# wenxichen/tensorflow_yolo2

Measured on AMD Instinct MI355X. Metric: images/sec fwd+bwd Darknet-19 416x416, higher is better.
Workload: dtype f16; 1 GPU; YOLO detector train step: darknet19_core + darknet19_detection(30) + get_loss + backward + Adam; image_size=416, batch_per_gpu=64, global_batch=64, S=13, B=2, parallelism=dp1, grad_allreduce=none

## Files before the change

tensorflow_yolo2_amd/csrc/common.h:

```cpp
#pragma once
#include <hip/hip_runtime.h>
#include <stdint.h>

namespace y2 {

typedef _Float16 half_t;
typedef __bf16 bf16_t;

typedef float f32x4 __attribute__((ext_vector_type(4)));
typedef float f32x16 __attribute__((ext_vector_type(16)));
typedef _Float16 f16x8 __attribute__((ext_vector_type(8)));
typedef _Float16 f16x4 __attribute__((ext_vector_type(4)));
typedef __bf16 bf16x8 __attribute__((ext_vector_type(8)));
typedef __bf16 bf16x4 __attribute__((ext_vector_type(4)));
typedef uint32_t u32x4 __attribute__((ext_vector_type(4)));
typedef uint32_t u32x2 __attribute__((ext_vector_type(2)));

#define Y2_DEV __device__ __forceinline__

constexpr int kWave = 64;

template <typename T> struct Elem;

template <> struct Elem<float> {
// ... 147 lines not shown
Y2_DEV float leaky01(float z) { return fmaxf(0.1f * z, z); }
Y2_DEV float leaky_s(float z, float s) { return fmaxf(s * z, z); }
Y2_DEV float leaky_slope_s(float z, float s) { return (s * z >= z) ? s : 1.0f; }
Y2_DEV float leaky01_slope(float z) { return (0.1f * z >= z) ? 0.1f : 1.0f; }

typedef short s16x4 __attribute__((__vector_size__(4 * sizeof(short))));
typedef short s16x8 __attribute__((ext_vector_type(8)));

template <typename T>
Y2_DEV typename Elem<T>::frag tr_frag(const char* p0, const char* p1) {
    s16x4 lo = __builtin_amdgcn_ds_read_tr16_b64_v4i16((__attribute__((address_space(3))) s16x4*)p0);
    s16x4 hi = __builtin_amdgcn_ds_read_tr16_b64_v4i16((__attribute__((address_space(3))) s16x4*)p1);
    s16x8 both = {lo[0], lo[1], lo[2], lo[3], hi[0], hi[1], hi[2], hi[3]};
    return __builtin_bit_cast(typename Elem<T>::frag, both);
}

__host__ __device__ inline size_t bpix(int n, int h, int w, int H, int W) {
    return ((size_t)n * (H + 1) + (size_t)(h + 1)) * (size_t)(W + 1) + (size_t)(w + 1);
}
__host__ __device__ inline size_t bbody_pixels(int N, int H, int W) {
    return (size_t)N * (H + 1) * (W + 1) + (size_t)(W + 1) + 1;
}

Y2_DEV int pool_order_pixel(int q, int H, int W) {
    const int Wo = W >> 1, Ho = H >> 1;
    const int win = q >> 2, d = q & 3;
    const int t = win / Wo, wo = win - t * Wo;
    const int n = t / Ho, ho = t - n * Ho;
    return (n * H + 2 * ho + (d >> 1)) * W + 2 * wo + (d & 1);
}

}
```

tensorflow_yolo2_amd/csrc/conv1_wgrad.hip:

```cpp
#include "common.h"
#include "kernels.h"

namespace y2 {

template <typename T>
__global__ __launch_bounds__(256) void conv1_wgrad_kernel(Conv1WgradArgs a) {
    constexpr int SZ = sizeof(T);
    constexpr int DYP = 32 * SZ;
    constexpr int XP = 4 * SZ;
    extern __shared__ __attribute__((aligned(16))) char smem[];
    const int tid = threadIdx.x, lane = tid & 63;
    const int w = __builtin_amdgcn_readfirstlane(tid >> 6);
    const int Wp = (a.W + 15) & ~15;
    const int dy_bytes = Wp * DYP;
    const int x_bytes = ((Wp + 4) * XP + 15) & ~15;
    char* dy_l = smem;
    char* x_l = smem + dy_bytes;
    const int dy_chunks = dy_bytes / 16, x_chunks = x_bytes / 16;
    const int rows = a.N * a.H;
    const int r32 = lane & 31, hh = lane >> 5;
    const int qq = (lane & 15) >> 2, pp = lane & 3, g1 = (lane >> 4) & 1;

    f32x16 acc1, acc2;
#pragma unroll
// ... 699 lines not shown
    for (int i = tid; i < 48 * 32; i += 1024) {
        const int r = i >> 5, co = i & 31;
        const int kh = r >> 4, e = r & 15, kw = e >> 2, c = e & 3;
        Wp[r][co] = (kw < 3 && c < 3) ? a.W[((kh * 3 + kw) * 3 + c) * 32 + co] : 0.f;
    }
    __syncthreads();
    if (tid >= 27 * 32) return;
    const int co = tid & 31, tc = tid >> 5;
    const int c = tc % 3, kw = (tc / 3) % 3, kh = tc / 9;
    const int r = kh * 16 + kw * 4 + c;
    constexpr int kOnes = 1 * 16 + 1 * 4 + 3;
    const float x1 = G[kOnes][r];
    float gw = 0.f;
    for (int k = 0; k < 48; ++k) gw = fmaf(G[r][k], Wp[k][co], gw);
    const float xy = gw + a.bias[co] * x1;
    const float xdz = total(r * 32 + co);
    const float ka = a.coef[co], kb = a.coef[32 + co];
    a.dW[tc * 32 + co] = (a.scale[co] * xdz - ka * x1 - kb * xy) * a.inv_grad_scale;
}

constexpr int kGram = 48 * 48;
constexpr int kGramMaxBlocks = 768;
template <typename T>
__global__ __launch_bounds__(256, 2) void conv1_gram_kernel(const void* x4, int N, int H, int W, int RT, float* part) {
    static_assert(sizeof(T) == 2, "half-precision modes only (the f32 parity mode keeps the statistics-only conv pass)");
    constexpr int SZ = 2, XP = 4 * SZ;
    constexpr int NTH = 256, NW = 4;
    typedef typename Elem<T>::frag frag_t;
    extern __shared__ __attribute__((aligned(16))) char smem[];
    const int tid = threadIdx.x, lane = tid & 63;
    const int w = __builtin_amdgcn_readfirstlane(tid >> 6);
    const int Wp = (W + 31) & ~31;
    const int x_bytes = ((Wp + 4) * XP + 15) & ~15;
    const int x_chunks = x_bytes / 16;
    const int nrow = RT + 2;
    char* x_l = smem;
    const int Ht = H / RT;
    const int ntile = N * Ht;
    const int g4 = lane >> 4, qq = (lane & 15) >> 2, pp = lane & 3;
    f32x4 gb[6];
#pragma unroll
    for (int k = 0; k < 6; ++k) gb[k] = f32x4{0.f, 0.f, 0.f, 0.f};
    auto stage = [&](int t, int buf) {
        const int n = t / Ht, h0 = (t - n * Ht) * RT;
        const char* xrow = (const char*)x4 + (bpix(n, h0, 0, H, W) - (size_t)(W + 2)) * XP;
        const size_t xpitch = (size_t)(W + 1) * XP;
        char* dst = x_l + buf * nrow * x_bytes;
        for (int kh = 0; kh < nrow; ++kh)
            for (int i0 = w * 64; i0 < x_chunks; i0 += NTH) {
                const int i = i0 + lane;
                if (i < x_chunks) glds16(xrow + kh * xpitch + (size_t)i * 16, dst + kh * x_bytes + i0 * 16);
            }
    };
    const int ngrp = (W + 31) / 32, nitem = ngrp * (RT / 2);
    int buf = 0;
    if ((int)blockIdx.x < ntile) stage(blockIdx.x, 0);
    for (int t = blockIdx.x; t < ntile; t += gridDim.x, buf ^= 1) {
        __syncthreads();
        if (t + (int)gridDim.x < ntile) stage(t + gridDim.x, buf ^ 1);
        const char* xb = x_l + buf * nrow * x_bytes;
        for (int it = w; it < nitem; it += NW) {
            const int s = it % ngrp, r0 = 2 * (it / ngrp);
            const int w0 = s * 32;
            const int pix = w0 + 8 * g4 + qq;
            frag_t X[4], B[4];
#pragma unroll
            for (int q = 0; q < 4; ++q) {
                const char* pa = xb + (r0 + q) * x_bytes + (pix + pp) * XP;
                X[q] = tr_frag<T>(pa, pa + 4 * XP);
                B[q] = X[q];
            }
            if (w0 + 32 > W) {
#pragma unroll
                for (int q = 0; q < 4; ++q)
#pragma unroll
                    for (int j = 0; j < 8; ++j)
                        if (w0 + 8 * g4 + j >= W) B[q][j] = (T)0.f;
            }
#pragma unroll
            for (int r = 0; r < 2; ++r) {
                mma16(gb[0], X[r], B[r]);
                mma16(gb[1], X[r], B[r + 1]);
                mma16(gb[2], X[r], B[r + 2]);
                mma16(gb[3], X[r + 1], B[r + 1]);
                mma16(gb[4], X[r + 1], B[r + 2]);
                mma16(gb[5], X[r + 2], B[r + 2]);
            }
        }
    }
    __syncthreads();
    float* red = (float*)smem;
    {
        float* g = red + w * kGram;
        const int bi[6] = {0, 0, 0, 1, 1, 2}, bj[6] = {0, 1, 2, 1, 2, 2};
#pragma unroll
        for (int k = 0; k < 6; ++k)
#pragma unroll
            for (int q = 0; q < 4; ++q) g[(bi[k] * 16 + 4 * g4 + q) * 48 + bj[k] * 16 + (lane & 15)] = gb[k][q];
    }
    __syncthreads();
    for (int i = tid; i < kGram; i += NTH) {
        const int r = i / 48, c = i % 48;
        const int j = (r / 16 > c / 16) ? c * 48 + r : i;
        part[(size_t)blockIdx.x * kGram + i] = (red[j] + red[kGram + j]) + (red[2 * kGram + j] + red[3 * kGram + j]);
    }
}

__global__ __launch_bounds__(256) void conv1_gram_reduce_kernel(const float* part, int nblocks, float* mid) {
    const int i = blockIdx.x * 256 + threadIdx.x;
    if (i >= kGram) return;
    const int per = (nblocks + kLinMid - 1) / kLinMid;
    const int b0 = blockIdx.y * per;
    int b1 = b0 + per;
    if (b1 > nblocks) b1 = nblocks;
    float v4[4] = {0.f, 0.f, 0.f, 0.f};
    int b = b0;
    for (; b + 3 < b1; b += 4)
#pragma unroll
        for (int u = 0; u < 4; ++u) v4[u] += part[(size_t)(b + u) * kGram + i];
    for (; b < b1; ++b) v4[0] += part[(size_t)b * kGram + i];
    mid[(size_t)blockIdx.y * kGram + i] = (v4[0] + v4[1]) + (v4[2] + v4[3]);
}

template <typename T>
__global__ __launch_bounds__(1024) void conv1_gram_stats_kernel(Conv1GramStatsArgs a) {
    __shared__ double G[48][49];
    __shared__ float Wq[48][32];
    __shared__ double t[48][33];
// ... 39 lines not shown
            s += sv[r] * (double)Wq[r][c];
        }
        if (m2 < 0) m2 = 0;
        const double mean = (double)a.bias[c] + s / M;
        const float var = (float)(M > 0 ? m2 / M : 0.0);
        const float meanf = (float)mean;
        const float inv = 1.0f / sqrtf(var + a.eps);
        const float sc = a.gamma[c] * inv;
        a.scale[c] = sc;
        a.shift[c] = a.beta[c] - meanf * sc;
        a.mean[c] = meanf;
        a.invstd[c] = inv;
        float vu = var;
        if (a.bessel && M > 1.0) vu = (float)(m2 / (M - 1.0));
        if (a.var) a.var[c] = vu;
        if (a.update_moving) {
            const float dec = 1.0f - a.momentum;
            a.moving_mean[c] -= (a.moving_mean[c] - meanf) * dec;
            a.moving_var[c] -= (a.moving_var[c] - vu) * dec;
        }
    }
}

template <typename T>
static hipError_t c1gram_T(const Conv1Plan& p, const Conv1GramStatsArgs& a, hipStream_t s) {
    if (p.gram_lds != c1gram_lds(p.gram_rt, a.Wd) || p.gram_lds > kC1LdsMax) return hipErrorInvalidValue;
    auto kern = conv1_gram_kernel<T>;
    static int attr = 0;
    if (p.gram_lds > attr) {
        hipError_t e = hipFuncSetAttribute((const void*)kern, hipFuncAttributeMaxDynamicSharedMemorySize, p.gram_lds);
        if (e != hipSuccess) return e;
        attr = p.gram_lds;
    }
    float* part = a.mid + (size_t)kLinMid * kGram;
    hipLaunchKernelGGL(kern, dim3(p.gram_blocks), dim3(256), p.gram_lds, s, a.x4, a.N, a.H, a.Wd, p.gram_rt, part);
    hipLaunchKernelGGL(conv1_gram_reduce_kernel, dim3((kGram + 255) / 256, kLinMid), dim3(256), 0, s, part, p.gram_blocks, a.mid);
    hipLaunchKernelGGL(conv1_gram_stats_kernel<T>, dim3(1), dim3(1024), 0, s, a);
    return hipGetLastError();
}
hipError_t launch_conv1_gram_stats(const Conv1Plan& p, const Conv1GramStatsArgs& a, hipStream_t s) {
    if (p.stats != C1S_GRAM) return hipErrorInvalidValue;
    switch (p.T) {
        case 1: return c1gram_T<half_t>(p, a, s);
        case 2: return c1gram_T<bf16_t>(p, a, s);
    }
    return hipErrorInvalidValue;
}

template <typename T, bool GRAM, bool NOSEL, int XS>
static hipError_t c1lin_T(const Conv1Plan& p, const Conv1WgradLinArgs& a0, hipStream_t s) {
    constexpr int SZ = sizeof(T);
    static_assert(c1lin_lds(2, 0) >= 2 * kLinThreads * (16 / SZ) * (int)sizeof(float), "the BN partial sums fit the LDS");
    const int wp = p.lin_nseg > 1 ? p.lin_ws : (a0.W + 15) & ~15;
    if (p.bwd_lds != c1lin_lds(XS == 2 ? 2 : SZ, wp) || p.bwd_lds > kC1LdsMax) return hipErrorInvalidValue;
    if (NOSEL && !(a0.Wf && a0.bias)) return hipErrorInvalidValue;
    Conv1WgradLinArgs a = a0;
    a.nseg = p.lin_nseg;
    a.ws = p.lin_ws;
// ... 25 lines not shown
        case c1lin_form(1, C1K_IDX3, 0, 0): return c1lin_T<half_t, false, true, 0>(p, a, s);
        case c1lin_form(2, C1K_IDX3, 0, 1): return c1lin_T<bf16_t, true, true, 0>(p, a, s);
        case c1lin_form(2, C1K_IDX3, 0, 0): return c1lin_T<bf16_t, false, true, 0>(p, a, s);
    }
    return hipErrorInvalidValue;
}
hipError_t launch_conv1_dw_finalize(const Conv1DwFinalizeArgs& a, hipStream_t s) {
    hipLaunchKernelGGL(conv1_dw_finalize_kernel, dim3(1), dim3(1024), 0, s, a);
    return hipGetLastError();
}

Conv1Plan plan_conv1(int dtype, int bwd_dtype, int N, int H, int W, int pool, int cout, int ldy, bool trains, bool has_next,
                     bool training) {
    Conv1Plan p{};
    const int sz = (int)dtype_size(dtype);
    const bool split = dtype_split(dtype);
    p.T = dtype_plain(dtype);
    const bool windows = pool && H % 2 == 0 && W % 2 == 0 && cout == 32 && ldy == 32;
    p.fwd = has_next && windows ? C1F_POOLED : C1F_PLAIN;
    const bool pooled = p.fwd == C1F_POOLED;
    const bool linear = trains && pooled && c1lin_lds(sz, (W + 15) & ~15) <= kC1LdsMax;
    const bool gram = linear && sz == 2 && 2 * c1_images(0, 6, (W + 31) & ~31, 2) <= 72 * 1024;
    p.stats = pooled && training ? (gram ? C1S_GRAM : C1S_CONV) : C1S_NONE;
    if (!pooled) p.keep = C1K_Y;
    else if (linear) p.keep = p.T == 0 && !split ? C1K_YSEL : C1K_IDX3;
    else p.keep = trains ? C1K_Y : C1K_NONE;
    p.xs_fwd = pooled && split && (linear || !trains) ? 1 : 0;
    p.xs_bwd = linear && split ? (bwd_dtype == 4 ? 2 : 1) : 0;
    p.lin_gram = linear && p.stats != C1S_GRAM ? 1 : 0;
    const bool fused = windows && c1wgf_lds(sz, W) <= kC1LdsMax;
    p.bwd = linear ? C1B_LINEAR : (pooled ? C1B_RECOMPUTE : (fused ? C1B_FUSED : C1B_GENERIC));

    const int nb = (N * H * W + 127) / 128;
    p.fwd_blocks = nb > 1024 ? 1024 : nb;
    const int tiles = N * (H / 2) * ((W + 31) / 32);
    p.pool_blocks = (tiles + 3) / 4 > 2048 ? 2048 : (tiles + 3) / 4;
    p.gram_rt = H % 4 == 0 ? 4 : 2;
    p.gram_blocks = N * (H / p.gram_rt) < kGramMaxBlocks ? N * (H / p.gram_rt) : kGramMaxBlocks;
    p.gram_lds = c1gram_lds(p.gram_rt, W);
    p.lin_nseg = 1;
    if (p.bwd == C1B_LINEAR) {
        const int isz = p.xs_bwd == 2 ? 2 : sz;
        int wp = (W + 15) & ~15;
        if (p.xs_bwd && c1_images(2, 4, wp, isz) > 80 * 1024) {
            const int ws = ((W + 1) / 2 + 15) & ~15;
            if (ws < W) p.lin_nseg = 2, p.lin_ws = wp = ws;
// ... 26 lines not shown
```

tensorflow_yolo2_amd/csrc/kernels.h:

```cpp
#pragma once
#include <hip/hip_runtime.h>
#include <stddef.h>
#include <stdint.h>
#include "../../include/yolo2_hip.h"

namespace y2 {

inline size_t dtype_size(int dtype) { return (dtype == 0 || dtype >= 3) ? 4 : 2; }
inline int dtype_kbytes(int dtype) { return dtype == 0 ? 4 : 2; }
inline bool dtype_split(int dtype) { return dtype >= 3; }
inline int dtype_plain(int dtype) { return dtype >= 3 ? 0 : dtype; }

struct ConvArgs {
    const void* x;
    const void* w;
    void* y;
    const float* bias;
    float* part_cnt;
    float* part_mean;
    float* part_m2;
    int N, H, W, C;
    int M;
    int Cout;
    int ldy;
// ... 106 lines not shown
    C1K_YSEL,
    C1K_IDX3,
};
enum Conv1Bwd {
    C1B_GENERIC,
    C1B_RECOMPUTE,
    C1B_FUSED,
    C1B_LINEAR,
};
struct Conv1Plan {
    int T;
    Conv1Fwd fwd;
    Conv1Stats stats;
    Conv1Keep keep;
    Conv1Bwd bwd;
    int xs_fwd;
    int xs_bwd;
    int lin_gram;
    int lin_nseg, lin_ws;
    int lin_records;
    int fwd_blocks;
    int pool_blocks;
    int gram_rt, gram_blocks, gram_lds;
    int bwd_blocks, bwd_lds;
    size_t ysel_bytes, idx_bytes, lin_bytes, gram_bytes;
    bool y_stored, dy_stored;
};
Conv1Plan plan_conv1(int dtype, int bwd_dtype, int N, int H, int W, int pool, int cout, int ldy, bool trains, bool has_next,
                     bool training);
constexpr int kC1LdsMax = 160 * 1024;
constexpr int c1_images(int dy_rows, int x_rows, int wp, int isz) {
    return dy_rows * wp * 32 * isz + x_rows * (((wp + 4) * 4 * isz + 15) & ~15);
}
constexpr int c1_atleast(int lds, int red) { return lds > red ? lds : red; }
constexpr int c1wg_lds(int sz, int W) { return c1_atleast(c1_images(1, 3, (W + 15) & ~15, sz), 4 * 48 * 32 * 4); }
constexpr int c1wgf_lds(int sz, int W) { return c1_atleast(c1_images(2, 4, (W + 15) & ~15, sz), 4 * 48 * 32 * 4); }
constexpr int c1lin_lds(int isz, int wp) { return c1_atleast(c1_images(2, 4, wp, isz), 4 * (48 * 32 + 48 * 48) * 4); }
constexpr int c1gram_lds(int rt, int W) { return c1_atleast(2 * c1_images(0, rt + 2, (W + 31) & ~31, 2), 4 * 48 * 48 * 4); }

struct Conv1Args {
    const void* x4;
    const void* w;
    void* y;
    const float* bias;
    float* part_cnt;
    float* part_mean;
// ... 61 lines not shown
};
struct Conv1DwFinalizeArgs {
    const float* acc;
    const float* W;
    const float* bias;
    const float* scale;
    const float* coef;
    float* dW;
    float inv_grad_scale;
    const float* gram = nullptr;
};
struct Conv1GramStatsArgs {
    const void* x4;
    int N, H, Wd;
    const float* W;
    const float* bias;
    const float *gamma, *beta;
    float *moving_mean, *moving_var;
    float *scale, *shift, *mean, *invstd, *var;
    float eps, momentum;
    int update_moving, bessel;
    float* mid;
    float* gram;
};
hipError_t launch_conv1_gram_stats(const Conv1Plan& p, const Conv1GramStatsArgs& a, hipStream_t s);
hipError_t launch_conv1_wgrad_lin(const Conv1Plan& p, const Conv1WgradLinArgs& a, hipStream_t s);
hipError_t launch_conv1_dw_finalize(const Conv1DwFinalizeArgs& a, hipStream_t s);

struct WgradArgs {
    const void* x;
    const void* dy;
    float* dW;
    int N, H, W, M;
    int Cin, Cdy, Cout;
    int taps;
    int splitk;
    float scale;
    int xcd = 0;
    float* slab = nullptr;
    size_t slab_floats = 0;
    int xpitch = 0, ypitch = 0;
    int quads = 1;
    int part0 = 0;
};
inline int wgrad_split_args(int dtype, WgradArgs& a) {
    if (!a.xpitch) a.xpitch = a.Cin;
// ... 93 lines not shown
hipError_t launch_pack_input_u8(int dtype, const uint8_t* img, void* x4, int N, int H, int W, hipStream_t s);
hipError_t launch_pack_weights(int dtype, const float* W, void* wf, void* wd, int taps, int Cin, int Cout,
                               int Cout_pad, int Kc, int Cin_pad, int Cdy, int frag, hipStream_t s);
hipError_t launch_pack_conv1_weights(int dtype, const float* W, void* wp, hipStream_t s);
struct PackLayer {
    const float* W;
    size_t w_off;
    void* wf;
    void* wd;
    int taps, Cin, Cout, Cout_pad, Kc, Cin_pad, Cdy;
    int wf_bx, wf_by, wf_blocks, wd_blocks, first_block;
    int opt_first;
    int wf_frag, wd_frag;
};
void pack_layer_plan(PackLayer& L, int first_block, int elem_size);
hipError_t launch_pack_all(int dtype, const PackLayer* tab_dev, int nlayers, int total_blocks, hipStream_t s);
struct OptPackArgs {
    float* p; float* slot0; float* slot1; const float* g;
    const void* ctrl;
    float lr_t, b1, b2, eps, gmult;
    int kind;
    const PackLayer* tab; int nlayers; int tile_blocks;
    const unsigned* small; int nsmall;
};
hipError_t launch_opt_pack(int dtype, const OptPackArgs& a, hipStream_t s);
hipError_t launch_convert_grad(int dtype, const float* src, void* dst, int M, int C, int ldd, float scale,
                               hipStream_t s);
hipError_t launch_unpack_act(int dtype, const void* xp, float* out, int N, int H, int W, int C, int Cs,
                             hipStream_t s);
hipError_t launch_pack_act_region(int dtype, const float* in, void* region, size_t region_bytes, size_t front_px, int N,
                                  int H, int W, int C, int Cs, hipStream_t s);
hipError_t launch_pack_act(int dtype, const float* in, void* xp, int N, int H, int W, int C, int Cs,
                           hipStream_t s);
hipError_t launch_cast_to_f32(int dtype, const void* src, float* dst, size_t rows, int C, int lds, hipStream_t s,
                              float scale = 1.0f);

struct BnFinalizeArgs {
    const float* part_cnt;
    const float* part_mean;
    const float* part_m2;
    int P, C, ldp;
    const float* gamma;
    const float* beta;
    float* moving_mean;
    float* moving_var;
    float* scale;
// ... 123 lines not shown
```

tensorflow_yolo2_amd/csrc/net.hip:

```cpp
#include <math.h>
#include <stdarg.h>
#include <stdio.h>
#include <string.h>

#include <algorithm>
#include <string>
#include <vector>

#include "../../include/yolo2_hip.h"
#include "common.h"
#include "kernels.h"
#include "optim_math.h"

using namespace y2;

static thread_local std::string g_err;
namespace y2 {
int set_error(int code, const char* msg) {
    g_err = msg;
    return code;
}
}
static int fail(int code, const char* fmt, ...) {
    char buf[512];
// ... 893 lines not shown
        int r = pack_all_weights(c, s);
        if (r) return r;
    }
    float* part_cnt = (float*)(c->ws + c->o_part_cnt);
    float* part_mean = (float*)(c->ws + c->o_part_mean);
    float* part_m2 = (float*)(c->ws + c->o_part_m2);
    const int nl = (int)c->L.size();
    c->fwd = plan_net(c, train_core, train_head, 0, 0);
    const Conv1Plan& p1 = c->fwd.c1;
    if (!train_core || (!train_head && c->core_layers < nl)) {
        int max_c = 0;
        for (const Layer& y : c->L) max_c = y.cout > max_c ? y.cout : max_c;
        HIPCHK(launch_bn_infer_prepare_all((const BnInferLayer*)(c->ws + c->o_infertab), nl, max_c, train_core, train_head,
                                           c->bn_eps, s));
    }
    for (int l = 0; l < nl; ++l) {
        c->prof_layer = l;
        const Layer& y = c->L[l];
        const LayerPlan& p = c->fwd.L[l];
        char* xin = (l == 0 && c->ext_xin) ? (char*)c->ext_xin : c->ws + y.xin + c->in_geom(l).base_off(sz);
        float* stat = (float*)(c->ws + y.stat);
        float *scale = stat, *shift = stat + y.ldy, *mean = stat + 2 * y.ldy, *invstd = stat + 3 * y.ldy;
        if (y.first3) {
            {
                PROF(CAT_MISC);
                if (images_u8) HIPCHK(launch_pack_input_u8(c->dtype, images_u8, xin, c->N, y.H, y.W, s));
                else HIPCHK(launch_pack_input(c->dtype, images, xin, c->N, y.H, y.W, s));
            }
            Conv1Args a{};
            a.x4 = xin; a.w = c->ws + y.wf; a.y = c->ws + y.y; a.bias = c->params + y.pb;
            a.part_cnt = part_cnt; a.part_mean = part_mean; a.part_m2 = part_m2;
            a.N = c->N; a.H = y.H; a.W = y.W; a.M = y.M;
            if (p.apply != FA_CONV1_POOL || p1.stats == C1S_CONV) { PROF(CAT_CONV1_FWD); HIPCHK(launch_conv1_fwd(p1, a, s)); }
        } else {
            if (l == 0 && !c->ext_xin) HIPCHK(launch_pack_act(c->dtype, images, xin, c->N, y.H, y.W, y.cin, y.cin_s, s));
            if (p.mx8) {
                const PadGeom g8{c->N, y.H, y.W, y.cin8}, gs{c->N, y.H, y.W, y.cin8 / 32};
                uint8_t* x8 = (uint8_t*)(c->ws + y.x8);
                uint8_t* x8s = (uint8_t*)(c->ws + y.x8s);
                if (!p.in8) {
                    PROF(CAT_MISC);
                    HIPCHK(launch_mx_quantize(1, xin - c->in_geom(l).base_off(sz), g8.front_px() + g8.body_px() + g8.back_px(),
                                              y.cin_s, y.cin8, x8, x8s, s));
                }
                ConvArgs a = fwd_args(c, l, false, p.fold);
                a.x = x8 + g8.base_off(1); a.C = y.cin8; a.w = c->ws + y.w8;
                a.ks_scratch = nullptr; a.ks_floats = 0;
// ... 16 lines not shown
            }
        }
        if (p.apply == FA_NONE) continue;
        PROF(CAT_BN_FWD);
        BnFinalizeArgs f{};
        if (p.training) {
            f.part_cnt = part_cnt; f.part_mean = part_mean; f.part_m2 = part_m2;
            f.P = p.P; f.C = y.cout; f.ldp = y.first3 ? 32 : y.ldy;
            f.gamma = c->params + y.pg; f.beta = c->params + y.pbeta;
            f.moving_mean = c->state + y.smm; f.moving_var = c->state + y.smv;
            f.scale = scale; f.shift = shift; f.mean = mean; f.invstd = invstd;
            f.var = stat + 6 * y.ldy;
            f.scratch = (float*)(c->ws + c->o_part_scratch);
            f.eps = c->bn_eps; f.momentum = c->bn_momentum; f.update_moving = update_moving ? 1 : 0; f.bessel = c->bessel;
        }
        if (p.stats == FS_GRAM) {
            Conv1GramStatsArgs q{};
            q.x4 = xin; q.N = c->N; q.H = y.H; q.Wd = y.W;
            q.W = c->params + y.pW; q.bias = c->params + y.pb; q.gamma = f.gamma; q.beta = f.beta;
            q.moving_mean = f.moving_mean; q.moving_var = f.moving_var;
            q.scale = scale; q.shift = shift; q.mean = mean; q.invstd = invstd; q.var = f.var;
            q.eps = f.eps; q.momentum = f.momentum; q.update_moving = f.update_moving; q.bessel = f.bessel;
            q.gram = (float*)(c->ws + c->o_gram); q.mid = q.gram + 48 * 48;
            HIPCHK(launch_conv1_gram_stats(p1, q, s));
        } else if (p.stats != FS_MOVING && p.apply != FA_FIN_ACT) {
            HIPCHK(launch_bn_finalize(f, s));
        }
        if (p.apply == FA_CONV1_POOL) {
            Conv1PoolArgs q{};
            q.x4 = xin; q.w = c->ws + y.wf; q.y = c->ws + y.y; q.bias = c->params + y.pb;
            q.scale = scale; q.shift = shift;
            q.out = c->ws + c->L[l + 1].xin + c->in_geom(l + 1).base_off(sz);
            q.N = c->N; q.H = y.H; q.W = y.W;
            q.out_split = dtype_split(c->dtype) ? 1 : 0;
            if (p1.keep == C1K_IDX3) q.idx3 = (unsigned*)(c->ws + y.idx0);
            if (p1.keep == C1K_YSEL) { q.ysel = c->ws + y.ysel; q.idx = (unsigned short*)(c->ws + y.idx0); }
            HIPCHK(launch_conv1_pool(p1, q, s));
            continue;
        }
        BnActArgs b{};
        b.y = c->ws + y.y; b.scale = scale; b.shift = shift;
        b.N = c->N; b.H = y.H; b.W = y.W; b.C = y.cout; b.ldy = y.ldy; b.pool = y.pool;
        b.slope = y.slope;
        const void* join_t = c->ext_join_self ? (const void*)(c->ext_xin ? (char*)c->ext_xin : c->ws + c->L[0].xin + c->in_geom(0).base_off(sz))
                                              : c->ext_join;
        switch (p.out) {
            case OUT_NEXT: b.out = c->ws + c->L[l + 1].xin + c->in_geom(l + 1).base_off(sz); break;
// ... 380 lines not shown
    if (!params || !m || !v || !grads || !ctrl) return fail(Y2_ERR_ARG, "bad arguments");
    HIPCHK(launch_opt_ctrl_advance(ctrl, lr, beta1, beta2, (hipStream_t)stream));
    HIPCHK(launch_adam_guarded(params, m, v, grads, n, ctrl, beta1, beta2, eps, grad_mult, (hipStream_t)stream));
    return Y2_OK;
}
int y2_momentum_step_guarded(float* params, float* accum, const float* grads, size_t n, void* ctrl, float lr,
                             float momentum, float grad_mult, void* stream) {
    if (!params || !accum || !grads || !ctrl) return fail(Y2_ERR_ARG, "bad arguments");
    HIPCHK(launch_opt_ctrl_advance(ctrl, lr, 0.9f, 0.999f, (hipStream_t)stream));
    HIPCHK(launch_momentum_guarded(params, accum, grads, n, ctrl, lr, momentum, grad_mult, (hipStream_t)stream));
    return Y2_OK;
}
static int opt_step_packed(y2_ctx* c, int kind, float* slot0, float* slot1, void* ctrl, float lr_t_or_lr, float b1,
                           float b2, float eps, float grad_mult, hipStream_t s, int part = 0) {
    if (!c->ws || !c->grads || !c->bound_training) return fail(Y2_ERR_STATE, "bind with training=1 first");
    OptPackArgs a{};
    a.p = c->params; a.slot0 = slot0; a.slot1 = slot1; a.g = c->grads; a.ctrl = ctrl;
    a.lr_t = lr_t_or_lr; a.b1 = b1; a.b2 = b2; a.eps = eps; a.gmult = grad_mult; a.kind = kind;
    a.tab = (const PackLayer*)(c->ws + c->o_packtab); a.nlayers = (int)c->packtab.size();
    a.tile_blocks = part == 2 ? 0 : c->opt_tile_blocks;
    const unsigned* small = (const unsigned*)(c->ws + c->o_smallranges);
    a.small = part == 2 ? small + 3 * c->n_small_upper : small;
    a.nsmall = part == 0 ? c->n_smallranges : (part == 1 ? c->n_small_upper : c->n_smallranges - c->n_small_upper);
    HIPCHK(launch_opt_pack(c->dtype, a, s));
    if (part != 1 && !c->L.empty() && c->L[0].first3)
        HIPCHK(launch_pack_conv1_weights(c->dtype, c->params + c->L[0].pW, c->ws + c->L[0].wf, s));
    if (part != 1) c->weights_dirty = false;
    return Y2_OK;
}
static int fused_opt_part(y2_ctx* c, int part, hipStream_t s) {
    const y2_ctx::FusedOpt& f = c->fopt;
    double lr_t = f.lr;
    if (f.ctrl) {
        if (part != 2) {
            const bool upper = part == 1;
            HIPCHK(launch_grad_check_ranges(c->grads, c->ws + c->o_chkranges, upper ? c->n_chk_upper : c->n_chkranges,
                                            f.ctrl, s, upper ? (unsigned*)(c->ws + c->o_nfflag) : nullptr));
            HIPCHK(launch_opt_ctrl_advance(f.ctrl, f.lr, f.kind == 0 ? f.b1 : 0.9f, f.kind == 0 ? f.b2 : 0.999f, s));
        }
    } else if (f.kind == 0) {
        lr_t = (double)f.lr * sqrt(1.0 - pow((double)f.b2, f.step)) / (1.0 - pow((double)f.b1, f.step));
    }
    return opt_step_packed(c, f.kind, f.slot0, f.slot1, f.ctrl, (float)lr_t, f.b1, f.b2, f.eps, f.gmult, s, part);
}
int y2_backward_adam(y2_ctx* c, const float* dout, float* m, float* v, void* ctrl, int step, float lr, float beta1,
                     float beta2, float eps, float grad_mult, void* stream) {
    if (c->fp8) return fail(Y2_ERR_STATE, "Y2_FP8 contexts are inference only: no backward pass (create the context with another dtype to train)");
    if (!m || !v || (!ctrl && step < 1)) return fail(Y2_ERR_ARG, "bad arguments");
    if (!c->grads) return fail(Y2_ERR_STATE, "bind with a gradient buffer first");
// ... 251 lines not shown
```

tensorflow_yolo2_amd/csrc/pack.hip:

```cpp
#include "common.h"
#include "kernels.h"
#include "optim_math.h"

namespace y2 {

template <typename T>
__global__ void pack_input_kernel(const float* __restrict__ img, T* __restrict__ x4, int N, int H, int W) {
    const size_t total = (size_t)N * H * W;
    for (size_t p = (size_t)blockIdx.x * blockDim.x + threadIdx.x; p < total; p += (size_t)gridDim.x * blockDim.x) {
        const int w = (int)(p % W);
        const int h = (int)((p / W) % H);
        const int n = (int)(p / ((size_t)W * H));
        const float* s = img + p * 3;
        T* d = x4 + bpix(n, h, w, H, W) * 4;
        d[0] = Elem<T>::from_f32(s[0]);
        d[1] = Elem<T>::from_f32(s[1]);
        d[2] = Elem<T>::from_f32(s[2]);
        d[3] = Elem<T>::from_f32(1.f);
    }
}
template <typename T>
static hipError_t pack_input_T(const float* img, void* x4, int N, int H, int W, hipStream_t s) {
    size_t total = (size_t)N * H * W;
    size_t nb = (total + 255) / 256;
    if (nb > 8192) nb = 8192;
    hipLaunchKernelGGL(pack_input_kernel<T>, dim3((unsigned)nb), dim3(256), 0, s, img, (T*)x4, N, H, W);
    return hipGetLastError();
}
Y2_DEV float u8_to_unit(uint32_t b) {
    float v = (float)b;
    v = __fdiv_rn(v, 255.0f);
    v = __fmul_rn(v, 2.0f);
    return __fsub_rn(v, 1.0f);
}
template <typename T>
__global__ void pack_input_u8_kernel(const uint8_t* __restrict__ img, T* __restrict__ x4, int N, int H, int W) {
    const size_t total = (size_t)N * H * W;
    const size_t quads = total / 4;
    for (size_t q = (size_t)blockIdx.x * blockDim.x + threadIdx.x; q < quads; q += (size_t)gridDim.x * blockDim.x) {
        const uint32_t* s = (const uint32_t*)(img + q * 12);
        const uint32_t w0 = s[0], w1 = s[1], w2 = s[2];
        const uint32_t by[12] = {w0 & 255u, (w0 >> 8) & 255u, (w0 >> 16) & 255u, w0 >> 24,
                                 w1 & 255u, (w1 >> 8) & 255u, (w1 >> 16) & 255u, w1 >> 24,
                                 w2 & 255u, (w2 >> 8) & 255u, (w2 >> 16) & 255u, w2 >> 24};
        size_t p = q * 4;
        int w = (int)(p % W);
        int h = (int)((p / W) % H);
        int n = (int)(p / ((size_t)W * H));
#pragma unroll
        for (int j = 0; j < 4; ++j) {
            T* d = x4 + bpix(n, h, w, H, W) * 4;
            T o[4] = {Elem<T>::from_f32(u8_to_unit(by[3 * j])), Elem<T>::from_f32(u8_to_unit(by[3 * j + 1])),
                      Elem<T>::from_f32(u8_to_unit(by[3 * j + 2])), Elem<T>::from_f32(1.f)};
            if (sizeof(T) == 2) *(u32x2*)d = *(const u32x2*)o;
            else *(u32x4*)d = *(const u32x4*)o;
            if (++w == W) { w = 0; if (++h == H) { h = 0; ++n; } }
// ... 504 lines not shown
    if (KIND == 0) adam_update(p, s0, s1, g, lr_t, b1, b2, eps);
    else if (KIND == 1) momentum_update(p, s0, g, lr_t, b1);
    else sgd_update(p, s0, g, lr_t, b1, b2, decayed);
}

template <typename T, int KIND, bool SPLIT = false>
__global__ __launch_bounds__(256) void opt_pack_kernel(OptPackArgs a) {
    constexpr int EPC = 16 / sizeof(T);
    constexpr int CPR = 64 / EPC;
    constexpr int RPP = 256 / CPR;
    float lr_t = a.lr_t;
    if (a.ctrl) {
        const OptCtrlView* c = (const OptCtrlView*)a.ctrl;
        if (c->found_inf) return;
        if (KIND != 1) lr_t = c->lr_t;
    }
    const int tid = threadIdx.x;
    const int b = blockIdx.x;
    if (b >= a.tile_blocks) {
        const int nb = gridDim.x - a.tile_blocks, bi = b - a.tile_blocks;
        for (int r = 0; r < a.nsmall; ++r) {
            const unsigned off = a.small[3 * r], cnt = a.small[3 * r + 1];
            const bool decayed = KIND == 2 && a.small[3 * r + 2] != 0;
            for (unsigned i = bi * 256 + tid; i < cnt; i += nb * 256) {
                float p = a.p[off + i], s0 = a.slot0[off + i], s1 = KIND == 0 ? a.slot1[off + i] : 0.f;
                opt_update<KIND>(p, s0, s1, a.g[off + i] * a.gmult, lr_t, a.b1, a.b2, a.eps, decayed);
                a.p[off + i] = p; a.slot0[off + i] = s0;
                if (KIND == 0) a.slot1[off + i] = s1;
            }
        }
        return;
    }
    __shared__ float tile[64][65];
    int l = 0;
    while (l + 1 < a.nlayers && b >= a.tab[l + 1].opt_first) ++l;
    const PackLayer L = a.tab[l];
    const int local = b - L.opt_first;
    const int bx = local % L.wf_bx, by = (local / L.wf_bx) % L.wf_by, t = local / (L.wf_bx * L.wf_by);
    const int ci0 = by * 64, co0 = bx * 64;
    const int c4 = (tid & 15) * 4, r0 = tid >> 4;
    const bool vec = (L.Cout & 3) == 0;
#pragma unroll
    for (int pass = 0; pass < 4; ++pass) {
        const int r = pass * 16 + r0;
        const int ci = ci0 + r, co = co0 + c4;
        float pv[4] = {0.f, 0.f, 0.f, 0.f};
        if (ci < L.Cin && co < L.Cout) {
            const size_t o = L.w_off + ((size_t)t * L.Cin + ci) * L.Cout + co;
            if (vec) {
                f32x4 p = *(const f32x4*)(a.p + o), s0 = *(const f32x4*)(a.slot0 + o), g = *(const f32x4*)(a.g + o);
                f32x4 s1 = KIND == 0 ? *(const f32x4*)(a.slot1 + o) : f32x4{0.f, 0.f, 0.f, 0.f};
// ... 127 lines not shown
```

Before: 7510 images/s.

## Fuse input packing into conv1 Gram stats kernel and conv1 weight pack into optimizer

Adds a conv1_gram_pack_kernel that reads raw float or u8 images, converts them to the padded 4-channel layout in LDS, writes the packed input to global memory as a side effect, and accumulates the Gram statistics in the same pass. This removes the separate pack_input launch and the re-read of the packed tensor by the Gram kernel. It also folds the conv1 weight repacking into the optimizer's small-range update loop, dropping another launch. Both fusions are on by default and can be disabled with an environment variable. The fused kernel has more complex index math and boundary handling, and its launch bounds change from 2 to 4 blocks per CU.

Result: no change. 7525 images/s, median of 4 (+0.2%).

```diff
diff --git a/tensorflow_yolo2_amd/csrc/common.h b/tensorflow_yolo2_amd/csrc/common.h
--- a/tensorflow_yolo2_amd/csrc/common.h
+++ b/tensorflow_yolo2_amd/csrc/common.h
@@ -193,6 +193,13 @@
     return (size_t)N * (H + 1) * (W + 1) + (size_t)(W + 1) + 1;
 }
 
+Y2_DEV float u8_to_unit(uint32_t b) {
+    float v = (float)b;
+    v = __fdiv_rn(v, 255.0f);
+    v = __fmul_rn(v, 2.0f);
+    return __fsub_rn(v, 1.0f);
+}
+
 Y2_DEV int pool_order_pixel(int q, int H, int W) {
     const int Wo = W >> 1, Ho = H >> 1;
     const int win = q >> 2, d = q & 3;
diff --git a/tensorflow_yolo2_amd/csrc/conv1_wgrad.hip b/tensorflow_yolo2_amd/csrc/conv1_wgrad.hip
--- a/tensorflow_yolo2_amd/csrc/conv1_wgrad.hip
+++ b/tensorflow_yolo2_amd/csrc/conv1_wgrad.hip
@@ -745,11 +745,66 @@
 constexpr int kGram = 48 * 48;
 constexpr int kGramMaxBlocks = 768;
 template <typename T>
+Y2_DEV void gram_tile_mma(const char* xb, int x_bytes, int W, int RT, int w, int lane, f32x4 (&gb)[6]) {
+    constexpr int XP = 8, NW = 4;
+    typedef typename Elem<T>::frag frag_t;
+    const int g4 = lane >> 4, qq = (lane & 15) >> 2, pp = lane & 3;
+    const int ngrp = (W + 31) / 32, nitem = ngrp * (RT / 2);
+    for (int it = w; it < nitem; it += NW) {
+        const int s = it % ngrp, r0 = 2 * (it / ngrp);
+        const int w0 = s * 32;
+        const int pix = w0 + 8 * g4 + qq;
+        frag_t X[4], B[4];
+#pragma unroll
+        for (int q = 0; q < 4; ++q) {
+            const char* pa = xb + (r0 + q) * x_bytes + (pix + pp) * XP;
+            X[q] = tr_frag<T>(pa, pa + 4 * XP);
+            B[q] = X[q];
+        }
+        if (w0 + 32 > W) {
+#pragma unroll
+            for (int q = 0; q < 4; ++q)
+#pragma unroll
+                for (int j = 0; j < 8; ++j)
+                    if (w0 + 8 * g4 + j >= W) B[q][j] = (T)0.f;
+        }
+#pragma unroll
+        for (int r = 0; r < 2; ++r) {
+            mma16(gb[0], X[r], B[r]);
+            mma16(gb[1], X[r], B[r + 1]);
+            mma16(gb[2], X[r], B[r + 2]);
+            mma16(gb[3], X[r + 1], B[r + 1]);
+            mma16(gb[4], X[r + 1], B[r + 2]);
+            mma16(gb[5], X[r + 2], B[r + 2]);
+        }
+    }
+}
+Y2_DEV void gram_block_partial(char* smem, int tid, int w, int lane, const f32x4 (&gb)[6], float* part) {
+    constexpr int NTH = 256;
+    const int g4 = lane >> 4;
+    __syncthreads();
+    float* red = (float*)smem;
+    {
+        float* g = red + w * kGram;
+        const int bi[6] = {0, 0, 0, 1, 1, 2}, bj[6] = {0, 1, 2, 1, 2, 2};
+#pragma unroll
+        for (int k = 0; k < 6; ++k)
+#pragma unroll
+            for (int q = 0; q < 4; ++q) g[(bi[k] * 16 + 4 * g4 + q) * 48 + bj[k] * 16 + (lane & 15)] = gb[k][q];
+    }
+    __syncthreads();
+    for (int i = tid; i < kGram; i += NTH) {
+        const int r = i / 48, c = i % 48;
+        const int j = (r / 16 > c / 16) ? c * 48 + r : i;
+        part[(size_t)blockIdx.x * kGram + i] = (red[j] + red[kGram + j]) + (red[2 * kGram + j] + red[3 * kGram + j]);
+    }
+}
+
+template <typename T>
 __global__ __launch_bounds__(256, 2) void conv1_gram_kernel(const void* x4, int N, int H, int W, int RT, float* part) {
     static_assert(sizeof(T) == 2, "half-precision modes only (the f32 parity mode keeps the statistics-only conv pass)");
     constexpr int SZ = 2, XP = 4 * SZ;
-    constexpr int NTH = 256, NW = 4;
-    typedef typename Elem<T>::frag frag_t;
+    constexpr int NTH = 256;
     extern __shared__ __attribute__((aligned(16))) char smem[];
     const int tid = threadIdx.x, lane = tid & 63;
     const int w = __builtin_amdgcn_readfirstlane(tid >> 6);
@@ -760,7 +815,6 @@
     char* x_l = smem;
     const int Ht = H / RT;
     const int ntile = N * Ht;
-    const int g4 = lane >> 4, qq = (lane & 15) >> 2, pp = lane & 3;
     f32x4 gb[6];
 #pragma unroll
     for (int k = 0; k < 6; ++k) gb[k] = f32x4{0.f, 0.f, 0.f, 0.f};
@@ -775,58 +829,139 @@
                 if (i < x_chunks) glds16(xrow + kh * xpitch + (size_t)i * 16, dst + kh * x_bytes + i0 * 16);
             }
     };
-    const int ngrp = (W + 31) / 32, nitem = ngrp * (RT / 2);
     int buf = 0;
     if ((int)blockIdx.x < ntile) stage(blockIdx.x, 0);
     for (int t = blockIdx.x; t < ntile; t += gridDim.x, buf ^= 1) {
         __syncthreads();
         if (t + (int)gridDim.x < ntile) stage(t + gridDim.x, buf ^ 1);
-        const char* xb = x_l + buf * nrow * x_bytes;
-        for (int it = w; it < nitem; it += NW) {
-            const int s = it % ngrp, r0 = 2 * (it / ngrp);
-            const int w0 = s * 32;
-            const int pix = w0 + 8 * g4 + qq;
-            frag_t X[4], B[4];
-#pragma unroll
-            for (int q = 0; q < 4; ++q) {
-                const char* pa = xb + (r0 + q) * x_bytes + (pix + pp) * XP;
-                X[q] = tr_frag<T>(pa, pa + 4 * XP);
-                B[q] = X[q];
-            }
-            if (w0 + 32 > W) {
-#pragma unroll
-                for (int q = 0; q < 4; ++q)
-#pragma unroll
-                    for (int j = 0; j < 8; ++j)
-                        if (w0 + 8 * g4 + j >= W) B[q][j] = (T)0.f;
-            }
-#pragma unroll
-            for (int r = 0; r < 2; ++r) {
-                mma16(gb[0], X[r], B[r]);
-                mma16(gb[1], X[r], B[r + 1]);
-                mma16(gb[2], X[r], B[r + 2]);
-                mma16(gb[3], X[r + 1], B[r + 1]);
-                mma16(gb[4], X[r + 1], B[r + 2]);
-                mma16(gb[5], X[r + 2], B[r + 2]);
-            }
-        }
-    }
-    __syncthreads();
-    float* red = (float*)smem;
-    {
-        float* g = red + w * kGram;
-        const int bi[6] = {0, 0, 0, 1, 1, 2}, bj[6] = {0, 1, 2, 1, 2, 2};
-#pragma unroll
-        for (int k = 0; k < 6; ++k)
-#pragma unroll
-            for (int q = 0; q < 4; ++q) g[(bi[k] * 16 + 4 * g4 + q) * 48 + bj[k] * 16 + (lane & 15)] = gb[k][q];
-    }
-    __syncthreads();
-    for (int i = tid; i < kGram; i += NTH) {
-        const int r = i / 48, c = i % 48;
-        const int j = (r / 16 > c / 16) ? c * 48 + r : i;
-        part[(size_t)blockIdx.x * kGram + i] = (red[j] + red[kGram + j]) + (red[2 * kGram + j] + red[3 * kGram + j]);
-    }
+        gram_tile_mma<T>(x_l + buf * nrow * x_bytes, x_bytes, W, RT, w, lane, gb);
+    }
+    gram_block_partial(smem, tid, w, lane, gb, part);
+}
+
+template <typename T, typename S>
+__global__ __launch_bounds__(256, 4) void conv1_gram_pack_kernel(const S* __restrict__ img, void* __restrict__ x4, int N,
+                                                                 int H, int W, int RT, float* part) {
+    static_assert(sizeof(T) == 2, "half-precision modes only");
+    constexpr bool U8 = sizeof(S) == 1;
+    constexpr int SZ = 2, XP = 4 * SZ;
+    constexpr int NTH = 256;
+    constexpr int PPU = U8 ? 4 : 1;
+    constexpr int KB = U8 ? 4 : 10;
+    extern __shared__ __attribute__((aligned(16))) char smem[];
+    const int tid = threadIdx.x, lane = tid & 63;
+    const int w = __builtin_amdgcn_readfirstlane(tid >> 6);
+    const int Wp = (W + 31) & ~31;
+    const int x_bytes = ((Wp + 4) * XP + 15) & ~15;
+    const int x_chunks = x_bytes / 16;
+    const int nrow = RT + 2;
+    char* x_l = smem;
+    const int Ht = H / RT;
+    const int ntile = N * Ht;
+    const float invW = 1.0f / (float)W;
+    const long long total_px = (long long)N * H * W;
+    f32x4 gb[6];
+#pragma unroll
+    for (int k = 0; k < 6; ++k) gb[k] = f32x4{0.f, 0.f, 0.f, 0.f};
+
+    struct Tile { int h0, d, ulo, uhi, jlo, jhi; long long base; const uint32_t* src; char* xdst; };
+    auto tile = [&](int t) {
+        Tile g;
+        const int n = t / Ht;
+        g.h0 = (t - n * Ht) * RT;
+        g.base = ((long long)n * H + g.h0 - 1) * W;
+        g.d = U8 ? (int)(g.base & 3) : 0;
+        g.ulo = g.h0 == 0 ? W : 0;
+        g.uhi = (g.h0 + RT == H ? RT + 1 : RT + 2) * W;
+        g.jlo = (g.ulo + g.d) / PPU;
+        g.jhi = (g.uhi - 1 + g.d) / PPU;
+        if constexpr (U8) {
+            const long long whole = (total_px - (g.base - g.d)) / 4 - 1;
+            if (whole < g.jhi) g.jhi = (int)whole;
+        }
+        g.src = (const uint32_t*)((const char*)img + (g.base - g.d) * 3 * (long long)sizeof(S));
+        g.xdst = (char*)x4 + (bpix(n, g.h0, 0, H, W) - (size_t)(W + 2)) * XP;
+        return g;
+    };
+    const int ldq = x_bytes - W * XP;
+    auto load_unit = [&](const Tile& g, int j, uint32_t (&r)[3]) {
+        asm volatile("" : "+v"(j));
+        const int jc = j < g.jlo ? g.jlo : (j > g.jhi ? g.jhi : j);
+        const uint32_t* s = g.src + 3u * (unsigned)jc;
+        r[0] = s[0]; r[1] = s[1]; r[2] = s[2];
+    };
+    auto put_unit = [&](const Tile& g, int j, const uint32_t (&r)[3], char* xb) {
+        asm volatile("" : "+v"(j));
+        const int u0 = j * PPU - g.d;
+        uint32_t rr[3] = {r[0], r[1], r[2]};
+        if constexpr (U8) {
+            if (j > g.jhi && u0 < g.uhi) {
+                const uint8_t* b = (const uint8_t*)(g.src + 3u * (unsigned)j);
+                const long long left = (total_px - (g.base + u0)) * 3;
+                rr[0] = rr[1] = rr[2] = 0u;
+#pragma unroll
+                for (int k = 0; k < 12; ++k)
+                    if (k < left) rr[k >> 2] |= (uint32_t)b[k] << (8 * (k & 3));
+            }
+        }
+#pragma unroll
+        for (int i = 0; i < PPU; ++i) {
+            const int u = u0 + i;
+            if (u < g.ulo || u >= g.uhi) continue;
+            int q = (int)((float)u * invW);
+            const int col = u - q * W;
+            if (col >= W) ++q;
+            else if (col < 0) --q;
+            float f[3];
+            if constexpr (!U8) {
+#pragma unroll
+                for (int e = 0; e < 3; ++e) f[e] = __builtin_bit_cast(float, rr[e]);
+            } else {
+#pragma unroll
+                for (int e = 0; e < 3; ++e) {
+                    const int k = 3 * i + e;
+                    f[e] = u8_to_unit((rr[k >> 2] >> (8 * (k & 3))) & 255u);
+                }
+            }
+            const T o[4] = {Elem<T>::from_f32(f[0]), Elem<T>::from_f32(f[1]), Elem<T>::from_f32(f[2]), Elem<T>::from_f32(1.f)};
+            const u32x2 v = *(const u32x2*)o;
+            *(u32x2*)(xb + (u + 1) * XP + q * ldq) = v;
+            if (q >= 1 && q <= RT) *(u32x2*)(g.xdst + (unsigned)(u + q + 1) * XP) = v;
+        }
+    };
+    for (int i = tid; i < 2 * nrow * x_chunks; i += NTH) *(u32x4*)(x_l + (size_t)i * 16) = u32x4{0, 0, 0, 0};
+    uint32_t raw[KB][3];
+    if ((int)blockIdx.x < ntile) {
+        const Tile g = tile(blockIdx.x);
+#pragma unroll
+        for (int k = 0; k < KB; ++k) load_unit(g, tid + k * NTH, raw[k]);
+    }
+    __syncthreads();
+    int buf = 0;
+    for (int t = blockIdx.x; t < ntile; t += gridDim.x, buf ^= 1) {
+        char* xb = x_l + buf * nrow * x_bytes;
+        const Tile g = tile(t);
+#pragma unroll
+        for (int k = 0; k < KB; ++k) put_unit(g, tid + k * NTH, raw[k], xb);
+        const int nunit = ((RT + 2) * W + g.d + PPU - 1) / PPU;
+        for (int j = tid + KB * NTH; j < nunit; j += NTH) {
+            uint32_t r[3];
+            load_unit(g, j, r);
+            put_unit(g, j, r, xb);
+        }
+        if (g.h0 == 0)
+            for (int i = tid; i < x_chunks; i += NTH) *(u32x4*)(xb + (size_t)i * 16) = u32x4{0, 0, 0, 0};
+        if (g.h0 + RT == H)
+            for (int i = tid; i < x_chunks; i += NTH) *(u32x4*)(xb + (RT + 1) * x_bytes + (size_t)i * 16) = u32x4{0, 0, 0, 0};
+        if (t + (int)gridDim.x < ntile) {
+            const Tile gn = tile(t + gridDim.x);
+#pragma unroll
+            for (int k = 0; k < KB; ++k) load_unit(gn, tid + k * NTH, raw[k]);
+        }
+        __syncthreads();
+        gram_tile_mma<T>(xb, x_bytes, W, RT, w, lane, gb);
+    }
+    gram_block_partial(smem, tid, w, lane, gb, part);
 }
 
 __global__ __launch_bounds__(256) void conv1_gram_reduce_kernel(const float* part, int nblocks, float* mid) {
@@ -912,6 +1047,21 @@
     }
 }
 
+template <typename T, typename S>
+static hipError_t c1gram_pack_launch(const Conv1Plan& p, const Conv1GramStatsArgs& a, const S* img, float* part, hipStream_t s) {
+    if (!img || !a.x4) return hipErrorInvalidValue;
+    if (sizeof(S) == 1 && ((uintptr_t)img & 3) != 0) return hipErrorInvalidValue;
+    auto kern = conv1_gram_pack_kernel<T, S>;
+    static int attr = 0;
+    if (p.gram_lds > attr) {
+        hipError_t e = hipFuncSetAttribute((const void*)kern, hipFuncAttributeMaxDynamicSharedMemorySize, p.gram_lds);
+        if (e != hipSuccess) return e;
+        attr = p.gram_lds;
+    }
+    hipLaunchKernelGGL(kern, dim3(p.gram_blocks), dim3(256), p.gram_lds, s, img, (void*)a.x4, a.N, a.H, a.Wd, p.gram_rt, part);
+    return hipSuccess;
+}
+
 template <typename T>
 static hipError_t c1gram_T(const Conv1Plan& p, const Conv1GramStatsArgs& a, hipStream_t s) {
     if (p.gram_lds != c1gram_lds(p.gram_rt, a.Wd) || p.gram_lds > kC1LdsMax) return hipErrorInvalidValue;
@@ -923,7 +1073,13 @@
         attr = p.gram_lds;
     }
     float* part = a.mid + (size_t)kLinMid * kGram;
-    hipLaunchKernelGGL(kern, dim3(p.gram_blocks), dim3(256), p.gram_lds, s, a.x4, a.N, a.H, a.Wd, p.gram_rt, part);
+    if (p.gram_pack) {
+        hipError_t e = a.img_u8 ? c1gram_pack_launch<T, uint8_t>(p, a, a.img_u8, part, s)
+                                : c1gram_pack_launch<T, float>(p, a, a.img, part, s);
+        if (e != hipSuccess) return e;
+    } else {
+        hipLaunchKernelGGL(kern, dim3(p.gram_blocks), dim3(256), p.gram_lds, s, a.x4, a.N, a.H, a.Wd, p.gram_rt, part);
+    }
     hipLaunchKernelGGL(conv1_gram_reduce_kernel, dim3((kGram + 255) / 256, kLinMid), dim3(256), 0, s, part, p.gram_blocks, a.mid);
     hipLaunchKernelGGL(conv1_gram_stats_kernel<T>, dim3(1), dim3(1024), 0, s, a);
     return hipGetLastError();
@@ -995,6 +1151,8 @@
     const bool linear = trains && pooled && c1lin_lds(sz, (W + 15) & ~15) <= kC1LdsMax;
     const bool gram = linear && sz == 2 && 2 * c1_images(0, 6, (W + 31) & ~31, 2) <= 72 * 1024;
     p.stats = pooled && training ? (gram ? C1S_GRAM : C1S_CONV) : C1S_NONE;
+    static const bool no_gram_pack = getenv("Y2_NO_GRAM_PACK") != nullptr;
+    p.gram_pack = p.stats == C1S_GRAM && !no_gram_pack ? 1 : 0;
     if (!pooled) p.keep = C1K_Y;
     else if (linear) p.keep = p.T == 0 && !split ? C1K_YSEL : C1K_IDX3;
     else p.keep = trains ? C1K_Y : C1K_NONE;
diff --git a/tensorflow_yolo2_amd/csrc/kernels.h b/tensorflow_yolo2_amd/csrc/kernels.h
--- a/tensorflow_yolo2_amd/csrc/kernels.h
+++ b/tensorflow_yolo2_amd/csrc/kernels.h
@@ -152,6 +152,7 @@
     int fwd_blocks;
     int pool_blocks;
     int gram_rt, gram_blocks, gram_lds;
+    int gram_pack;
     int bwd_blocks, bwd_lds;
     size_t ysel_bytes, idx_bytes, lin_bytes, gram_bytes;
     bool y_stored, dy_stored;
@@ -259,6 +260,8 @@
     int update_moving, bessel;
     float* mid;
     float* gram;
+    const float* img = nullptr;
+    const uint8_t* img_u8 = nullptr;
 };
 hipError_t launch_conv1_gram_stats(const Conv1Plan& p, const Conv1GramStatsArgs& a, hipStream_t s);
 hipError_t launch_conv1_wgrad_lin(const Conv1Plan& p, const Conv1WgradLinArgs& a, hipStream_t s);
@@ -398,6 +401,7 @@
     int kind;
     const PackLayer* tab; int nlayers; int tile_blocks;
     const unsigned* small; int nsmall;
+    void* c1_wp = nullptr; unsigned c1_off = 0;
 };
 hipError_t launch_opt_pack(int dtype, const OptPackArgs& a, hipStream_t s);
 hipError_t launch_convert_grad(int dtype, const float* src, void* dst, int M, int C, int ldd, float scale,
diff --git a/tensorflow_yolo2_amd/csrc/net.hip b/tensorflow_yolo2_amd/csrc/net.hip
--- a/tensorflow_yolo2_amd/csrc/net.hip
+++ b/tensorflow_yolo2_amd/csrc/net.hip
@@ -939,7 +939,7 @@
         float* stat = (float*)(c->ws + y.stat);
         float *scale = stat, *shift = stat + y.ldy, *mean = stat + 2 * y.ldy, *invstd = stat + 3 * y.ldy;
         if (y.first3) {
-            {
+            if (!(p.stats == FS_GRAM && p1.gram_pack && !c->ext_xin)) {
                 PROF(CAT_MISC);
                 if (images_u8) HIPCHK(launch_pack_input_u8(c->dtype, images_u8, xin, c->N, y.H, y.W, s));
                 else HIPCHK(launch_pack_input(c->dtype, images, xin, c->N, y.H, y.W, s));
@@ -1002,7 +1002,10 @@
             q.scale = scale; q.shift = shift; q.mean = mean; q.invstd = invstd; q.var = f.var;
             q.eps = f.eps; q.momentum = f.momentum; q.update_moving = f.update_moving; q.bessel = f.bessel;
             q.gram = (float*)(c->ws + c->o_gram); q.mid = q.gram + 48 * 48;
-            HIPCHK(launch_conv1_gram_stats(p1, q, s));
+            Conv1Plan pg = p1;
+            if (c->ext_xin) pg.gram_pack = 0;
+            if (pg.gram_pack) { q.img = images; q.img_u8 = images_u8; }
+            HIPCHK(launch_conv1_gram_stats(pg, q, s));
         } else if (p.stats != FS_MOVING && p.apply != FA_FIN_ACT) {
             HIPCHK(launch_bn_finalize(f, s));
         }
@@ -1429,9 +1432,14 @@
     const unsigned* small = (const unsigned*)(c->ws + c->o_smallranges);
     a.small = part == 2 ? small + 3 * c->n_small_upper : small;
     a.nsmall = part == 0 ? c->n_smallranges : (part == 1 ? c->n_small_upper : c->n_smallranges - c->n_small_upper);
+    static const bool c1_separate = getenv("Y2_NO_GRAM_PACK") != nullptr;
+    const bool c1 = part != 1 && !c->L.empty() && c->L[0].first3;
+    if (c1 && !c1_separate) {
+        a.c1_wp = c->ws + c->L[0].wf;
+        a.c1_off = (unsigned)c->L[0].pW;
+    }
     HIPCHK(launch_opt_pack(c->dtype, a, s));
-    if (part != 1 && !c->L.empty() && c->L[0].first3)
-        HIPCHK(launch_pack_conv1_weights(c->dtype, c->params + c->L[0].pW, c->ws + c->L[0].wf, s));
+    if (c1 && c1_separate) HIPCHK(launch_pack_conv1_weights(c->dtype, c->params + c->L[0].pW, c->ws + c->L[0].wf, s));
     if (part != 1) c->weights_dirty = false;
     return Y2_OK;
 }
diff --git a/tensorflow_yolo2_amd/csrc/pack.hip b/tensorflow_yolo2_amd/csrc/pack.hip
--- a/tensorflow_yolo2_amd/csrc/pack.hip
+++ b/tensorflow_yolo2_amd/csrc/pack.hip
@@ -26,12 +26,6 @@
     if (nb > 8192) nb = 8192;
     hipLaunchKernelGGL(pack_input_kernel<T>, dim3((unsigned)nb), dim3(256), 0, s, img, (T*)x4, N, H, W);
     return hipGetLastError();
-}
-Y2_DEV float u8_to_unit(uint32_t b) {
-    float v = (float)b;
-    v = __fdiv_rn(v, 255.0f);
-    v = __fmul_rn(v, 2.0f);
-    return __fsub_rn(v, 1.0f);
 }
 template <typename T>
 __global__ void pack_input_u8_kernel(const uint8_t* __restrict__ img, T* __restrict__ x4, int N, int H, int W) {
@@ -582,11 +576,18 @@
         for (int r = 0; r < a.nsmall; ++r) {
             const unsigned off = a.small[3 * r], cnt = a.small[3 * r + 1];
             const bool decayed = KIND == 2 && a.small[3 * r + 2] != 0;
+            const bool conv1 = a.c1_wp != nullptr && off == a.c1_off;
             for (unsigned i = bi * 256 + tid; i < cnt; i += nb * 256) {
                 float p = a.p[off + i], s0 = a.slot0[off + i], s1 = KIND == 0 ? a.slot1[off + i] : 0.f;
                 opt_update<KIND>(p, s0, s1, a.g[off + i] * a.gmult, lr_t, a.b1, a.b2, a.eps, decayed);
                 a.p[off + i] = p; a.slot0[off + i] = s0;
                 if (KIND == 0) a.slot1[off + i] = s1;
+                if (conv1) {
+                    const unsigned co = i & 31u, tc = i >> 5, c = tc % 3u, kw = (tc / 3u) % 3u, kh = tc / 9u;
+                    const unsigned o = co * 48u + kh * 16u + kw * 4u + c;
+                    if constexpr (SPLIT) ((float*)a.c1_wp)[o] = p;
+                    else ((T*)a.c1_wp)[o] = Elem<T>::from_f32(p);
+                }
             }
         }
         return;
```
